# darglein/Snake-SLAM

Measured on AMD Instinct MI355X. Metric: frames/s ORB extract+match @752x480, higher is better.
Workload: dtype u8

## Files before the change

### include/snake_hip.h

```cpp
#ifndef SNAKE_HIP_H
#define SNAKE_HIP_H

#include <stddef.h>
#include <stdint.h>

#ifdef __cplusplus
extern "C" {
#endif

#define SNK_API __attribute__((visibility("default")))

typedef enum snk_status
{
    SNK_OK                = 0,
    SNK_ERR_INVALID_ARG   = 1,
    SNK_ERR_NO_DEVICE     = 2,
    SNK_ERR_HIP           = 3,
    SNK_ERR_CAPACITY      = 4,
    SNK_ERR_NOT_CONFIGURED = 5,
    SNK_ERR_TIMEOUT       = 6
} snk_status;

#define SNK_DIST_INF 256

// ... 84 lines not shown
                                     int out_cap);

SNK_API int snk_orb_set_profiling(snk_orb* o, int enable);

SNK_API int snk_orb_set_chains(snk_orb* o, int chains);
SNK_API int snk_orb_set_stagger(snk_orb* o, int parts);
SNK_API int snk_orb_stage_times(snk_orb* o, float* ms, int* n_calls);

enum
{
    SNK_ORB_DEBUG_PYRAMID         = 1,
    SNK_ORB_DEBUG_CELL_COUNTS     = 2,
    SNK_ORB_DEBUG_CELL_CANDIDATES = 3,
    SNK_ORB_DEBUG_SELECTED        = 4,
    SNK_ORB_DEBUG_SELECTED_COUNT  = 5,
    SNK_ORB_DEBUG_LEVEL_INFO      = 6
};
SNK_API int snk_orb_debug_fetch(snk_orb* o, int what, int image, int level, void* out, size_t cap_bytes,
                                size_t* n_bytes);


typedef struct snk_rectification
{
    double K_src[4];
    double D_src[8];
    double R[9];
    double K_dst[4];
    double bf;
} snk_rectification;

SNK_API int snk_rectify(snk_matcher* m, const snk_rectification* rect, const snk_keypoint* kps, int n, snk_kp64* out,
// ... 557 lines not shown
```

### snake_slam_amd/csrc/orb.hip

```cpp
#include "common.hpp"

#include <array>
#include <vector>

namespace snk
{
namespace
{
using u8  = unsigned char;
using u16 = unsigned short;
using u32 = unsigned int;
using u64 = unsigned long long;

constexpr int MAX_LEVELS     = 16;
constexpr int EDGE_THRESHOLD = 19;
constexpr int MIN_BORDER     = 16;
constexpr int CELL_W         = 30;
constexpr int CELL_SLOTS     = 64;
constexpr int KEY_DIGITS     = 16;
constexpr int DEFAULT_LEVEL_CAP = 8192;
#ifndef SNK_DIST_MIN_WAVES
#define SNK_DIST_MIN_WAVES 1
#endif
#ifndef SNK_FAST_MIN_WAVES
// ... 1056 lines not shown
                    }
                    if (out_lane && !no_blur_store)
                    {
                        const u32 lo = __builtin_amdgcn_perm(a[1], a[0], 0x0c0c0602u);
                        const u32 hi = __builtin_amdgcn_perm(a[3], a[2], 0x06020c0cu);
                        *reinterpret_cast<u32*>(blur + (blur_tiled ? blur_tiled_y(yo, bpitch) : (u32)(yo * bpitch)) + xl_store) = lo | hi;
                    }
                }
#pragma unroll
                for (int c = 0; c < 4; ++c) pr[kk][c] = __builtin_amdgcn_alignbit(hc[c], pr[(kk + 6) % 7][c], 16);
            }
        }
    }
}

__device__ __forceinline__ u64 point_key(int x, int y, int W, int H, int nroots)
{
    const u32 ux = (u32)x, uw = (u32)W, un = (u32)nroots;
    const int root = (int)((ux * un) / uw);
    int x0 = (int)(((u32)root * uw + un - 1u) / un), x1 = (int)(((u32)(root + 1) * uw + un - 1u) / un);
    int y0 = 0, y1 = H;
    u64 key = (u64)root;
    const int ext = max(max(W, H), 2);
    const int nd  = min(KEY_DIGITS, 32 - __clz(ext - 1));
    for (int d = 0; d < nd; ++d)
    {
        const int mx = x0 + (x1 - x0 + 1) / 2, my = y0 + (y1 - y0 + 1) / 2;
        const int cx = x >= mx, cy = y >= my;
        x0 = cx ? mx : x0;
        x1 = cx ? x1 : mx;
        y0 = cy ? my : y0;
        y1 = cy ? y1 : my;
        key = (key << 2) | (u64)(cx + 2 * cy);
    }
    return key << (2 * (KEY_DIGITS - nd));
}

__device__ void bitonic_sort(u64* a, int n_pow2, int tid, int nthreads)
{
    const int nw = nthreads >> 6, wave = tid >> 6, lane = tid & 63;
    const int seg = n_pow2 / nw;
    if (seg < 128)
    {
        for (int k = 2; k <= n_pow2; k <<= 1)
            for (int j = k >> 1; j > 0; j >>= 1)
            {
                for (int t = tid; t < (n_pow2 >> 1); t += nthreads)
                {
                    const int i   = ((t & ~(j - 1)) << 1) | (t & (j - 1));
                    const int ixj = i | j;
// ... 39 lines not shown
                const bool up = (i & k) == 0;
                const u64 x = a[i], y = a[ixj];
                if ((x > y) == up)
                {
                    a[i]   = y;
                    a[ixj] = x;
                }
            }
            __builtin_amdgcn_wave_barrier();
        }
    }
    __syncthreads();
}

constexpr int DIST_THREADS = 512;
__device__ int block_scan_incl(int v, int tid, int* wave_tot )
{
    const int lane = tid & 63, wave = tid >> 6;
    int x = v;
    x = wave_scan_incl_dpp(x);
    if (lane == 63) wave_tot[wave] = x;
    __syncthreads();
    int base = 0;
    for (int w = 0; w < wave; ++w) base += wave_tot[w];
    __syncthreads();
    return x + base;
}

__device__ void bucket_rank_sort(u64* keys, int n, int cap, int nroots, unsigned char* tmp, int tid, int* wave_tot)
{
    u16* idx  = reinterpret_cast<u16*>(tmp);
    int* hist = reinterpret_cast<int*>(tmp + 2 * cap);
    const int nb_max = min(1023, cap / 2 - 1);
    int T = 4;
    while (T > 0 && (nroots << (2 * T)) > nb_max) --T;
    const int nb    = nroots << (2 * T);
    const int shift = 13 + 32 - 2 * T;
    for (int i = tid; i <= nb; i += DIST_THREADS) hist[i] = 0;
    __syncthreads();
    for (int i = tid; i < n; i += DIST_THREADS) atomicAdd(&hist[(int)(keys[i] >> shift)], 1);
    __syncthreads();
    {
        const int b0 = 2 * tid, c0 = b0 < nb ? hist[b0] : 0, c1 = b0 + 1 < nb ? hist[b0 + 1] : 0;
        const int incl = block_scan_incl(c0 + c1, tid, wave_tot);
        if (b0 < nb) hist[b0] = incl - c0 - c1;
        if (b0 + 1 < nb) hist[b0 + 1] = incl - c1;
    }
    __syncthreads();
    for (int i = tid; i < n; i += DIST_THREADS) idx[atomicAdd(&hist[(int)(keys[i] >> shift)], 1)] = (u16)i;
    __syncthreads();
    u64 mine[4];
    int dest[4];
#pragma unroll
    for (int u = 0; u < 4; ++u)
    {
        const int i = tid + u * DIST_THREADS;
        mine[u] = 0;
        dest[u] = -1;
        if (i < n)
// ... 15 lines not shown
    }
    __syncthreads();
#pragma unroll
    for (int u = 0; u < 4; ++u)
        if (dest[u] >= 0) keys[dest[u]] = mine[u];
    __syncthreads();
}

__device__ bool distribute_body(const Layout& L, int b, int l, int lds_cap, u32* cand ,
                                const u16* __restrict__ cell_cnt, u32* __restrict__ sel ,
                                u8* __restrict__ sel_score, int* __restrict__ sel_cnt,
                                int* __restrict__ cand_total ,
                                unsigned long long* __restrict__ dbg_t = nullptr ,
                                u32* cand_h = nullptr ,
                                u32* __restrict__ sel_resp = nullptr ,
                                u32* __restrict__ h_global = nullptr )
{
    extern __shared__ __attribute__((aligned(16))) unsigned char smem[];
    const int cap     = lds_cap;
    const int sem_cap = L.level_cap;
    u64* keys     = reinterpret_cast<u64*>(smem);
    u64* nodes    = keys + cap;
    u16* px       = reinterpret_cast<u16*>(nodes + cap / 2);
    u16* py       = px + cap;
    u8* sc        = reinterpret_cast<u8*>(py + cap);
    signed char* lcp = reinterpret_cast<signed char*>(sc + cap);
    u8* fd        = reinterpret_cast<u8*>(lcp + cap + 16);
    u32* hv       = cand_h ? (h_global ? h_global : reinterpret_cast<u32*>(smem + ((cap * 8 + cap / 2 * 8 + cap * 2 * 2 + cap + (cap + 16) + cap + 15) & ~15)))
                           : nullptr;
    __shared__ int wave_tot[8];
    __shared__ int hist_lcp[20], hist_m[20];
    __shared__ int s_n, s_k, s_D, s_careful, s_size, s_nnodes, s_finish, s_jstar, s_out;

    const int tid = threadIdx.x;
    unsigned long long t_prev = dbg_t ? __builtin_readcyclecounter() : 0ull;
    auto mark = [&](int phase)
    {
        if (dbg_t && tid == 0)
        {
            const unsigned long long t = __builtin_readcyclecounter();
            atomicAdd(&dbg_t[l * 16 + phase], t - t_prev);
            t_prev = t;
        }
    };
    const LevelInfo& lv = L.lv[l];
    const int ncell = lv.ncols * lv.nrows;
    const int N     = lv.nfeat;
    const u16* cc   = cell_cnt + (long long)b * L.total_cells + lv.cell_off;
    u32* cd         = cand + ((long long)b * L.total_cells + lv.cell_off) * CELL_SLOTS;
    u32* chd        = cand_h ? cand_h + ((long long)b * L.total_cells + lv.cell_off) * CELL_SLOTS : nullptr;
    int* out_cnt    = sel_cnt + b * MAX_LEVELS + l;

    if (tid == 0) s_k = CELL_SLOTS;
    __syncthreads();
    for (;;)
    {
        const int k = s_k;
        int part    = 0;
        for (int c = tid; c < ncell; c += DIST_THREADS) part += min((int)cc[c], k);
        const int incl = block_scan_incl(part, tid, wave_tot);
        if (tid == DIST_THREADS - 1) s_n = incl;
        __syncthreads();
        if (s_n <= sem_cap || k == 0) break;
        if (tid == 0) s_k = k - 1;
        __syncthreads();
    }
    const int kcell = s_k;
    const int n     = s_n;
    mark(0);
    if (n > cap) return false;
    if (kcell < CELL_SLOTS)
    {
        u32* cdw = cd;
        u32* chw = chd;
        const int lane = tid & 63;
        for (int c = tid >> 6; c < ncell; c += DIST_THREADS / 64)
        {
            const int cnt = (int)cc[c];
            if (cnt <= kcell || cnt > CELL_SLOTS) continue;
            const u32 k = lane < cnt ? cdw[(long long)c * CELL_SLOTS + lane] : 0u;
            const u32 h = chw && lane < cnt ? chw[(long long)c * CELL_SLOTS + lane] : 0u;
            int r       = 0;
            for (int j = 0; j < cnt; ++j) r += (u32)__builtin_amdgcn_readlane((int)k, __builtin_amdgcn_readfirstlane(j)) > k ? 1 : 0;
// ... 8 lines not shown
    }
    if (tid == 0 && cand_total) cand_total[b * MAX_LEVELS + l] = n;
    if (n == 0 || N <= 0)
    {
        if (tid == 0) *out_cnt = 0;
        return true;
    }
    int n_pow2 = 1;
    while (n_pow2 < n) n_pow2 <<= 1;

    {
        int base = 0;
        for (int c0 = 0; c0 < ncell; c0 += DIST_THREADS)
        {
            const int c   = c0 + tid;
            const int cnt = c < ncell ? min((int)cc[c], kcell) : 0;
            const int incl = block_scan_incl(cnt, tid, wave_tot);
            const int off  = base + incl - cnt;
            if (cnt > 0)
            {
                const int ci = c / lv.ncols, cj = c - ci * lv.ncols;
                const int x0 = EDGE_THRESHOLD + cj * lv.wcell, y0 = EDGE_THRESHOLD + ci * lv.hcell;
                const uint4* cq = reinterpret_cast<const uint4*>(cd + (long long)c * CELL_SLOTS);
                for (int i = 0; i < cnt; i += 32)
                {
                    uint4 q[8];
#pragma unroll
                    for (int v = 0; v < 8; ++v) q[v] = i + 4 * v < cnt ? cq[(i >> 2) + v] : uint4{0u, 0u, 0u, 0u};
#pragma unroll
                    for (int v = 0; v < 8; ++v)
                    {
                        const u32 kk[4] = {q[v].x, q[v].y, q[v].z, q[v].w};
#pragma unroll
                        for (int u = 0; u < 4; ++u)
                            if (i + 4 * v + u < cnt)
                            {
                                const u32 k = kk[u];
                                const int o = off + i + 4 * v + u;
                                px[o] = (u16)(x0 + 63 - (int)(k & 63u));
                                py[o] = (u16)(y0 + 63 - (int)((k >> 6) & 63u));
                                sc[o] = (u8)(k >> 12);
                                if (hv) hv[o] = chd[(long long)c * CELL_SLOTS + i + 4 * v + u];
                            }
                    }
                }
            }
            if (tid == DIST_THREADS - 1) s_out = incl;
            __syncthreads();
            base += s_out;
            __syncthreads();
        }
    }
    mark(1);
    const int W = lv.w - 2 * MIN_BORDER, H = lv.h - 2 * MIN_BORDER;
    for (int i = tid; i < n_pow2; i += DIST_THREADS)
        keys[i] = i < n ? ((point_key(px[i] - MIN_BORDER, py[i] - MIN_BORDER, W, H, lv.nroots) << 13) | (u64)i) : ~0ull;
    __syncthreads();

    mark(2);
    if (n <= 4 * DIST_THREADS && cap >= 512)
        bucket_rank_sort(keys, n, cap, lv.nroots, reinterpret_cast<unsigned char*>(nodes), tid, wave_tot);
    else
        bitonic_sort(keys, n_pow2, tid, DIST_THREADS);
    mark(3);

    if (tid < 20)
    {
        hist_lcp[tid] = 0;
        hist_m[tid]   = 0;
    }
    for (int i = tid; i <= n; i += DIST_THREADS)
    {
        int v = -1;
        if (i > 0 && i < n)
        {
            const u64 diff = (keys[i] >> 13) ^ (keys[i - 1] >> 13);
// ... 31 lines not shown
            const int multi = size - cum_m;
            if (size >= N || size == size_prev)
            {
                D = d; careful = 0; size_D = size; done = true;
            }
            else if (size + 3 * multi > N)
            {
                D = d; careful = 1; size_D = size; done = true;
            }
            size_prev = size;
            if (!done && d == KEY_DIGITS) { D = KEY_DIGITS; careful = 0; size_D = size; }
        }
        s_D       = D;
        s_careful = careful;
        s_size    = size_D;
        s_finish  = 0;
    }
    __syncthreads();
    const int D = s_D;
    for (int i = tid; i < n; i += DIST_THREADS) fd[i] = (u8)D;
    __syncthreads();

    mark(5);
    if (s_careful && n <= 4 * DIST_THREADS)
    {
        int* hist = reinterpret_cast<int*>(nodes);
        const int HN = n - 1;
        for (int dd = D; dd < KEY_DIGITS; ++dd)
        {
            for (int k = tid; k < HN; k += DIST_THREADS) hist[k] = 0;
            if (tid == 0) s_jstar = HN;
            if (dbg_t && tid == 0) atomicAdd(&dbg_t[l * 16 + 14], 1ull);
            __syncthreads();
            int cntv[4], delv[4];
            bool any = false;
#pragma unroll
            for (int u = 0; u < 4; ++u)
            {
                const int i = 4 * tid + u;
                cntv[u] = delv[u] = 0;
                if (i < n && fd[i] == dd && (int)lcp[i] < dd)
                {
                    int e = i + 1, delta = 0;
                    for (;;)
                    {
                        const int l0 = lcp[e], l1 = lcp[e + 1], l2 = lcp[e + 2], l3 = lcp[e + 3];
// ... 13 lines not shown
                }
            }
            mark(8);
            if (!__syncthreads_or(any ? 1 : 0)) break;
            mark(9);
            int before_mine = 0;
            {
                int loc[4], sum = 0;
#pragma unroll
                for (int u = 0; u < 4; ++u)
                {
                    const int k = 4 * tid + u;
                    loc[u]      = k < HN ? hist[HN - 1 - k] : 0;
                    sum += loc[u];
                }
                const int incl = block_scan_incl(sum, tid, wave_tot);
                int run        = s_size + incl - sum;
                int found      = -1;
#pragma unroll
                for (int u = 0; u < 4; ++u)
                {
                    if (found < 0 && loc[u] > 0 && run + loc[u] >= N) { found = 4 * tid + u; before_mine = run; }
                    run += loc[u];
                }
                if (found >= 0) atomicMin(&s_jstar, found);
                if (tid == DIST_THREADS - 1) s_out = run - s_size;
            }
            __syncthreads();
            mark(10);
            const int kstar = s_jstar;
            if (kstar < HN && 4 * tid <= kstar && kstar < 4 * tid + 4) s_nnodes = before_mine;
            __syncthreads();
            const int cstar  = kstar < HN ? HN - 1 - kstar + 2 : 0;
            const int before = kstar < HN ? s_nnodes : 0;
            int my_add = 0;
            bool split[4];
#pragma unroll
            for (int u = 0; u < 4; ++u) split[u] = cntv[u] > 0 && (cstar == 0 || cntv[u] > cstar);
            if (cstar != 0)
            {
                int d[4], sum = 0;
#pragma unroll
                for (int u = 0; u < 4; ++u)
                {
                    d[u] = cntv[u] == cstar ? delv[u] : 0;
                    sum += d[u];
                }
                int run = before + block_scan_incl(sum, tid, wave_tot) - sum;
#pragma unroll
                for (int u = 0; u < 4; ++u)
                {
                    if (cntv[u] == cstar && run < N) split[u] = true;
                    run += d[u];
                }
            }
#pragma unroll
            for (int u = 0; u < 4; ++u)
                if (split[u]) my_add += delv[u];
            mark(11);
            const int add = block_scan_incl(my_add, tid, wave_tot);
            if (tid == DIST_THREADS - 1)
            {
                s_finish = (s_size + add >= N || add == 0) ? 1 : 0;
                s_size += add;
            }
#pragma unroll
            for (int u = 0; u < 4; ++u)
                if (split[u])
                    for (int e = 4 * tid + u, e1 = e + cntv[u]; e < e1; ++e) fd[e] = (u8)(dd + 1);
            __syncthreads();
            mark(12);
            if (s_finish) break;
        }
    }
    else if (s_careful)
    {
        for (int dd = D; dd < KEY_DIGITS; ++dd)
        {
            if (tid == 0) s_nnodes = 0;
            __syncthreads();
            for (int i = tid; i < n; i += DIST_THREADS)
            {
                if (fd[i] != dd || (int)lcp[i] >= dd) continue;
                int e = i + 1, delta = 0;
                while (e < n && (int)lcp[e] >= dd)
                {
                    delta += (int)lcp[e] == dd ? 1 : 0;
// ... 4 lines not shown
                {
                    const u64 nk = ((u64)(0xFFFF - cnt) << 32) | ((u64)i << 16) | (u64)delta;
                    nodes[atomicAdd(&s_nnodes, 1)] = nk;
                }
            }
            __syncthreads();
            const int m = s_nnodes;
            if (m == 0) break;
            int m_pow2 = 1;
            while (m_pow2 < m) m_pow2 <<= 1;
            for (int i = m + tid; i < m_pow2; i += DIST_THREADS) nodes[i] = ~0ull;
            __syncthreads();
            bitonic_sort(nodes, m_pow2, tid, DIST_THREADS);
            if (tid == 0) s_jstar = m;
            __syncthreads();
            int base = s_size;
            for (int j0 = 0; j0 < m; j0 += DIST_THREADS)
            {
                const int j     = j0 + tid;
                const int delta = j < m ? (int)(nodes[j] & 0xFFFFu) : 0;
                const int incl  = block_scan_incl(delta, tid, wave_tot);
                if (j < m && base + incl >= N) atomicMin(&s_jstar, j);
                if (tid == DIST_THREADS - 1) s_out = incl;
                __syncthreads();
                base += s_out;
                __syncthreads();
            }
            const int jstar = s_jstar;
            const int last  = jstar < m ? jstar : m - 1;
            {
                int part = 0;
                for (int j = tid; j <= last; j += DIST_THREADS) part += (int)(nodes[j] & 0xFFFFu);
                const int add = block_scan_incl(part, tid, wave_tot);
                if (tid == DIST_THREADS - 1)
                {
                    s_finish = (s_size + add >= N || add == 0) ? 1 : 0;
                    s_size += add;
                }
            }
            for (int j = tid; j <= last; j += DIST_THREADS)
            {
                const int i = (int)((nodes[j] >> 16) & 0xFFFFu);
                int e       = i;
                do
                {
                    fd[e] = (u8)(dd + 1);
                    ++e;
                } while (e < n && (int)lcp[e] >= dd);
            }
            __syncthreads();
            if (s_finish) break;
        }
    }
    __syncthreads();

    mark(6);
    {
        u32* out    = sel + (long long)b * L.total_slots + lv.slot_off;
        u8* out_sc  = sel_score + (long long)b * L.total_slots + lv.slot_off;
        for (int i = tid; i < n; i += DIST_THREADS)
        {
            const int c = (int)(keys[i] & 0x1FFFu);
            keys[i]     = ((u64)(hv ? hv[c] : (u32)sc[c]) << 32) | ((u64)(0xFFFFu - py[c]) << 16) | (u64)(0xFFFFu - px[c]);
        }
        __syncthreads();
        unsigned long long* best = reinterpret_cast<unsigned long long*>(nodes);
        const int best_cap = min(n, lv.slot_cap);
        for (int k = tid; k < best_cap; k += DIST_THREADS) best[k] = 0ull;
        __syncthreads();
        int base = 0;
        for (int i0 = 0; i0 < n; i0 += DIST_THREADS)
        {
            const int i     = i0 + tid;
            const bool head = i < n && (int)lcp[i] < (int)fd[i];
            const int incl  = block_scan_incl(head ? 1 : 0, tid, wave_tot);
            const int pos   = base + incl - 1;
            if (i < n && pos < best_cap) atomicMax(&best[pos], (unsigned long long)keys[i]);
            if (tid == DIST_THREADS - 1) s_out = incl;
            __syncthreads();
            base += s_out;
            __syncthreads();
        }
        const int count = base < lv.slot_cap ? base : lv.slot_cap;
        for (int k = tid; k < count; k += DIST_THREADS)
        {
            const unsigned long long w = best[k];
            out[k]    = (0xFFFFu - (u32)(w & 0xFFFFu)) | ((0xFFFFu - (u32)((w >> 16) & 0xFFFFu)) << 16);
            out_sc[k] = (u8)(w >> 32);
            if (sel_resp) sel_resp[(long long)b * L.total_slots + lv.slot_off + k] = (u32)(w >> 32);
        }
        if (tid == 0) *out_cnt = count;
    }
    mark(7);
    if (dbg_t && tid == 0) atomicAdd(&dbg_t[l * 16 + 15], (unsigned long long)n);
    return true;
}

__global__ __launch_bounds__(DIST_THREADS, SNK_DIST_MIN_WAVES) void distribute_kernel(Layout L, int lds_cap, u32* cand,
                                                                  const u16* __restrict__ cell_cnt, u32* __restrict__ sel,
                                                                  u8* __restrict__ sel_score, int* __restrict__ sel_cnt,
                                                                  int* __restrict__ cand_total, int* __restrict__ queue,
                                                                  unsigned long long* __restrict__ dbg_t, u32* cand_h,
                                                                  u32* __restrict__ sel_resp)
{
    const int l = blockIdx.x, b = blockIdx.y;
    if (!distribute_body(L, b, l, lds_cap, cand, cell_cnt, sel, sel_score, sel_cnt, cand_total, dbg_t, cand_h, sel_resp) && threadIdx.x == 0)
        queue[1 + atomicAdd(&queue[0], 1)] = b * MAX_LEVELS + l;
}

__global__ __launch_bounds__(DIST_THREADS) void distribute_large_kernel(Layout L, u32* cand,
                                                                        const u16* __restrict__ cell_cnt,
                                                                        u32* __restrict__ sel, u8* __restrict__ sel_score,
                                                                        int* __restrict__ sel_cnt, int* __restrict__ cand_total,
                                                                        const int* __restrict__ queue, u32* cand_h,
                                                                        u32* __restrict__ sel_resp, u32* __restrict__ h_scratch)
{
    const int count = queue[0];
    for (int i = blockIdx.x; i < count; i += gridDim.x)
    {
        const int item = queue[1 + i];
        distribute_body(L, item / MAX_LEVELS, item % MAX_LEVELS, L.level_cap, cand, cell_cnt, sel, sel_score, sel_cnt, cand_total, nullptr,
                        cand_h, sel_resp, cand_h ? h_scratch + (size_t)blockIdx.x * L.level_cap : nullptr);
        __syncthreads();
    }
}

__device__ __forceinline__ float fast_atan2_deg(float y, float x)
{
    const float p1 = 0x1.ca44dep+5f, p3 = -0x1.2aaddcp+4f, p5 = 0x1.1d3f7ep+3f, p7 = -0x1.4515b2p+1f;
    const float ax = fabsf(x), ay = fabsf(y);
    float a, c, c2;
    if (ax >= ay)
    {
        c  = ay / (ax + 0x1p-52f);
        c2 = c * c;
        a  = (((p7 * c2 + p5) * c2 + p3) * c2 + p1) * c;
    }
// ... 439 lines not shown
}
}

using namespace snk;

struct snk_orb : HandleBase
{
    snk_orb_params params{};
    int width = 0, height = 0, max_batch = 0;
    bool configured = false;
    Layout lay{};
    DevBuf pyr[MAX_LEVELS];
    DevBuf blur[MAX_LEVELS];
    DevBuf tables;
    DevBuf cell_tab;
    DevBuf img0;
    DevBuf cand, cell_cnt, sel, sel_score, sel_cnt, cand_total, dist_queue;
    DevBuf cand_h, sel_resp, dist_h;
    DevBuf out_kps;
    HostBuf h_out, h_img;
    int pitch0_host = 0;
    size_t dist_lds = 0, dist_lds_small = 0;
    int dist_small_cap = 0;
    bool profiling = false;
    std::vector<std::array<hipEvent_t, 7>> ev_sets;
    size_t ev_used = 0;
    static constexpr int MAX_PARTS = 4;
    hipStream_t stream2 = nullptr;
    hipStream_t extra[MAX_PARTS - 1] = {nullptr, nullptr, nullptr};
    hipEvent_t ev_fork = nullptr, ev_join_n[MAX_PARTS - 1] = {nullptr, nullptr, nullptr};
// ... 37 lines not shown
        const int width = lv.w - 2 * MIN_BORDER, height = lv.h - 2 * MIN_BORDER;
        lv.ncols = width > 0 ? width / CELL_W : 0;
        lv.nrows = height > 0 ? height / CELL_W : 0;
        if (lv.ncols < 1 || lv.nrows < 1 || lv.w < 2 * EDGE_THRESHOLD + 1 || lv.h < 2 * EDGE_THRESHOLD + 1)
        {
            lv.ncols = lv.nrows = 0;
            lv.wcell = lv.hcell = 1;
        }
        else
        {
            lv.wcell = (width + lv.ncols - 1) / lv.ncols;
            lv.hcell = (height + lv.nrows - 1) / lv.nrows;
        }
        lv.cell_off = cell_off;
        cell_off += lv.ncols * lv.nrows;
        int nroots = height > 0 ? (2 * width + height) / (2 * height) : 1;
        nroots     = nroots < 1 ? 1 : (nroots > 255 ? 255 : nroots);
        lv.nroots  = nroots;
        lv.slot_off = slot_off;
        lv.slot_cap = lv.nfeat + 3 > 4 * nroots ? lv.nfeat + 3 : 4 * nroots;
        slot_off += lv.slot_cap;
        lv.pitch      = (lv.w + 63) & ~63;
        lv.img_stride = (long long)lv.pitch * lv.h;
        lv.blur_stride = (long long)lv.pitch * ((lv.h + 3) & ~3);
        if (lv.w > 0 && lv.h > 0)
        {
            static const bool balanced = getenv("SNK_ORB_BALANCED_STRIPS") != nullptr;
            if (balanced || lv.w <= 4 * SM_LANES_OUT)
            {
                lv.n_strips     = ceil_div(lv.w, 4 * SM_LANES_OUT);
                lv.strip_stride = ((ceil_div(lv.w, lv.n_strips) + 3) / 4) * 4;
            }
            else
// ... 123 lines not shown
    *out = o;
    return SNK_OK;
}

int snk_orb_destroy(snk_orb* o)
{
    if (!o) return SNK_OK;
    (void)hipSetDevice(o->device);
    for (auto& b : o->pyr) b.release();
    for (auto& b : o->blur) b.release();
    o->tables.release();
    o->img0.release();
    o->cand.release();
    o->cell_cnt.release();
    o->cell_tab.release();
    o->sel.release();
    o->sel_score.release();
    o->sel_cnt.release();
    o->cand_total.release();
    o->dist_queue.release();
    o->cand_h.release();
    o->sel_resp.release();
    o->dist_h.release();
    o->out_kps.release();
    o->h_out.release();
    o->h_img.release();
    for (auto& e : o->ev_sets)
        for (auto& x : e) (void)hipEventDestroy(x);
    if (o->ev_fork) (void)hipEventDestroy(o->ev_fork);
    for (auto& e : o->ev_front)
// ... 88 lines not shown
                const int ci = c / lv.ncols, cj = c - ci * lv.ncols;
                const int x0 = EDGE_THRESHOLD + cj * lv.wcell, y0 = EDGE_THRESHOLD + ci * lv.hcell;
                const int x1 = std::min(x0 + lv.wcell, lv.w - EDGE_THRESHOLD), y1 = std::min(y0 + lv.hcell, lv.h - EDGE_THRESHOLD);
                int4 e;
                e.x = x0;
                e.y = y0;
                e.z = (int)(((unsigned)(x1 - x0) & 0xFFFFu) | ((unsigned)(y1 - y0) << 16));
                e.w = l;
                ct[(size_t)lv.cell_off + c] = e;
            }
        }
        if ((rc = o->cell_tab.reserve(ct.size() * sizeof(int4))) != SNK_OK) return rc;
        if ((rc = copy_sync(o->cell_tab.p, ct.data(), ct.size() * sizeof(int4), hipMemcpyHostToDevice, o->stream)) != SNK_OK) return rc;
        L.cell_tab = o->cell_tab.as<int4>();
    }
    const size_t cells = (size_t)(L.total_cells > 0 ? L.total_cells : 1) * max_batch;
    const size_t slots = (size_t)(L.total_slots > 0 ? L.total_slots : 1) * max_batch;
    if ((rc = o->cand.reserve(cells * CELL_SLOTS * sizeof(u32))) != SNK_OK) return rc;
    if ((rc = o->cell_cnt.reserve(cells * sizeof(u16))) != SNK_OK) return rc;
    if ((rc = o->sel.reserve(slots * sizeof(u32))) != SNK_OK) return rc;
    if ((rc = o->sel_score.reserve(slots)) != SNK_OK) return rc;
    if ((rc = o->sel_cnt.reserve((size_t)max_batch * MAX_LEVELS * sizeof(int))) != SNK_OK) return rc;
    if ((rc = o->cand_total.reserve((size_t)max_batch * MAX_LEVELS * sizeof(int))) != SNK_OK) return rc;
    auto dist_lds_bytes = [](size_t cap) { return cap * 8 + cap / 2 * 8 + cap * 2 * 2 + cap + (cap + 16) + cap; };
    o->dist_small_cap = L.level_cap < 2048 ? L.level_cap : 2048;
    o->dist_lds       = dist_lds_bytes((size_t)L.level_cap);
    o->dist_lds_small = dist_lds_bytes((size_t)o->dist_small_cap);
    if ((rc = o->dist_queue.reserve(snk_orb::MAX_PARTS * ((size_t)max_batch * MAX_LEVELS + 1) * sizeof(int))) != SNK_OK) return rc;
    SNK_REQUIRE(4 * L.f_lds_wave <= LDS_MAX_BYTES, "FAST cells too large for the LDS (image too small for its cell grid?)");
    if ((rc = set_max_lds_once(reinterpret_cast<const void*>(distribute_kernel), (int)std::max(dist_lds_bytes(2048) + 4 * 2048 + 16, dist_lds_bytes(8192)))) != SNK_OK) return rc;
// ... 142 lines not shown
        static const size_t lds_wg_env = getenv("SNK_ORB_FAST_LDS_WG") ? (size_t)atoll(getenv("SNK_ORB_FAST_LDS_WG")) : 0;
        const size_t fast_lds = std::max((size_t)4 * L.f_lds_wave, std::min(lds_wg_env, (size_t)LDS_MAX_BYTES));
        hipLaunchKernelGGL(fk, xcd_grid(gx, batch), dim3(256), fast_lds, st, L, images_dev, pitch,
                           image_stride, aligned0, o->params.ini_th_fast, o->params.min_th_fast, d_cand, d_cellcnt, gx, batch, fast_stop,
                           cpw, stages == 3 ? d_queue : (int*)nullptr);
        SNK_LAUNCH_CHECK();
    }
    if (ev) SNK_HIP_CHECK(hipEventRecord((*ev)[3], st));
    }
    if (!(stages & 2)) return SNK_OK;
    if (ev) SNK_HIP_CHECK(hipEventRecord((*ev)[6], st));
    {
    const int aligned0 = (reinterpret_cast<uintptr_t>(images_dev) % 4 == 0 && pitch % 4 == 0 && image_stride % 4 == 0) ? 1 : 0;
    if (stages != 3 || L.total_cells <= 0) SNK_HIP_CHECK(hipMemsetAsync(d_queue, 0, sizeof(int), st));
    static const bool dist_timing = getenv("SNK_ORB_DIST_TIMING") != nullptr;
    unsigned long long* d_dbg = nullptr;
    if (dist_timing)
    {
        SNK_HIP_CHECK(hipMalloc(&d_dbg, MAX_LEVELS * 16 * sizeof(unsigned long long)));
        SNK_HIP_CHECK(hipMemsetAsync(d_dbg, 0, MAX_LEVELS * 16 * sizeof(unsigned long long), st));
    }
    if (harris && L.total_cells > 0)
    {
        static const bool per_cell = getenv("SNK_ORB_HARRIS_PER_CELL") != nullptr;
        if (per_cell)
        {
            const int gxh = ceil_div(L.total_cells, 4);
            hipLaunchKernelGGL(harris_kernel, xcd_grid(gxh, batch), dim3(256), 0, st, L, images_dev, pitch, image_stride, aligned0, d_cand, d_cellcnt,
                               d_candh, gxh, batch);
        }
        else
        {
            const int gxh = ceil_div(ceil_div(L.total_cells, HARRIS_NC), 4);
            hipLaunchKernelGGL(harris_dense_kernel, xcd_grid(gxh, batch), dim3(256), 0, st, L, images_dev, pitch, image_stride, aligned0, d_cand,
                               d_cellcnt, d_candh, gxh, batch);
        }
        SNK_LAUNCH_CHECK();
    }
    const bool one_dist_launch = !harris && o->dist_small_cap < L.level_cap && (long long)L.n_levels * batch <= 128;
    hipLaunchKernelGGL(distribute_kernel, dim3(L.n_levels, batch), dim3(DIST_THREADS),
                       one_dist_launch ? o->dist_lds : o->dist_lds_small + (harris ? 4 * (size_t)o->dist_small_cap + 16 : 0), st, L,
                       one_dist_launch ? L.level_cap : o->dist_small_cap, d_cand, d_cellcnt, d_sel, d_selscore,
                       d_selcnt, d_candtot, d_queue, d_dbg, d_candh, d_selresp);
    SNK_LAUNCH_CHECK();
    if (dist_timing)
    {
        unsigned long long h[MAX_LEVELS * 16];
        SNK_HIP_CHECK(hipStreamSynchronize(st));
        SNK_HIP_CHECK(hipMemcpy(h, d_dbg, sizeof(h), hipMemcpyDeviceToHost));
        SNK_HIP_CHECK(hipFree(d_dbg));
        for (int l = 0; l < L.n_levels; ++l)
        {
            fprintf(stderr, "[dist timing] level %d (avg candidates %.0f, %.2f careful rounds), cycles per workgroup:", l,
                    (double)h[l * 16 + 15] / batch, (double)h[l * 16 + 14] / batch);
            for (int ph = 0; ph < 13; ++ph) fprintf(stderr, " %.0f", (double)h[l * 16 + ph] / batch);
            fprintf(stderr, "\n");
        }
    }
    if (o->dist_small_cap < L.level_cap && !one_dist_launch)
    {
        hipLaunchKernelGGL(distribute_large_kernel, dim3(large_workers), dim3(DIST_THREADS), o->dist_lds, st, L,
                           d_cand, d_cellcnt, d_sel, d_selscore,
                           d_selcnt, d_candtot, d_queue, d_candh, d_selresp, d_disth);
        SNK_LAUNCH_CHECK();
    }
    if (ev) SNK_HIP_CHECK(hipEventRecord((*ev)[4], st));
    int max_slot = 1;
    for (int l = 0; l < L.n_levels; ++l) max_slot = L.lv[l].slot_cap > max_slot ? L.lv[l].slot_cap : max_slot;
    {
        const int nb = batch >= 16 ? 8 * ceil_div(batch, 8) : batch;
        static const bool blur_in = getenv("SNK_ORB_BLUR_IN_DESCRIBE") != nullptr;
        static const bool dma = getenv("SNK_ORB_DESC_NO_DMA") == nullptr;
        const int dfake       = getenv("SNK_ORB_DESC_FAKE") ? atoi(getenv("SNK_ORB_DESC_FAKE")) : 0;
        const int gx          = ceil_div(max_slot, 4 * DESC_KPW);
        auto dk = describe_kernel<false, false, false>;
        if (blur_in) dk = describe_kernel<true, false, false>;
        else if (dma && orb_blur_mode() == 2) dk = describe_kernel<false, true, true>;
        else if (dma) dk = describe_kernel<false, true, false>;
// ... 206 lines not shown
            src   = o->cell_cnt.as<u16>() + (long long)image * L.total_cells + lv.cell_off;
            bytes = (size_t)lv.ncols * lv.nrows * sizeof(u16);
            break;
        case SNK_ORB_DEBUG_CELL_CANDIDATES:
            src   = o->cand.as<u32>() + ((long long)image * L.total_cells + lv.cell_off) * CELL_SLOTS;
            bytes = (size_t)lv.ncols * lv.nrows * CELL_SLOTS * sizeof(u32);
            break;
        case SNK_ORB_DEBUG_SELECTED:
            src   = o->sel.as<u32>() + (long long)image * L.total_slots + lv.slot_off;
            bytes = (size_t)lv.slot_cap * sizeof(u32);
            break;
        case SNK_ORB_DEBUG_SELECTED_COUNT:
            src   = o->sel_cnt.as<int>() + image * MAX_LEVELS + level;
            bytes = sizeof(int);
            break;
        case SNK_ORB_DEBUG_LEVEL_INFO:
        {
            int info[8] = {lv.w, lv.h, lv.pitch, lv.ncols, lv.nrows, lv.wcell, lv.hcell, lv.nfeat};
            SNK_REQUIRE(cap_bytes >= sizeof(info), "buffer too small");
            memcpy(out, info, sizeof(info));
            *n_bytes = sizeof(info);
            return SNK_OK;
        }
        default: SNK_REQUIRE(false, "unknown debug selector");
    }
    SNK_REQUIRE(out != nullptr && cap_bytes >= bytes, "buffer too small");
    if (int rc = copy_sync(out, src, bytes, hipMemcpyDeviceToHost, o->stream)) return rc;
    *n_bytes = bytes;
    return SNK_OK;
}
// ... 2 lines not shown
```

### snake_slam_amd/orb.py

```python
from __future__ import annotations

import ctypes as C

import numpy as np

from . import _lib

KEYPOINT_DTYPE = np.dtype([("x", "<f4"), ("y", "<f4"), ("size", "<f4"), ("angle", "<f4"), ("response", "<f4"),
                           ("octave", "<i4")])

DEBUG_PYRAMID, DEBUG_CELL_COUNTS, DEBUG_CELL_CANDIDATES, DEBUG_SELECTED, DEBUG_SELECTED_COUNT, DEBUG_LEVEL_INFO = range(1, 7)


class OrbParams(C.Structure):
    _fields_ = [("nfeatures", C.c_int32), ("scale_factor", C.c_float), ("n_levels", C.c_int32),
                ("ini_th_fast", C.c_int32), ("min_th_fast", C.c_int32), ("level_cap", C.c_int32)]


class ORBExtractor:
    def __init__(self, nfeatures: int = 1000, scale_factor: float = 1.2, n_levels: int = 4, ini_th_fast: int = 20,
                 min_th_fast: int = 7, level_cap: int = 0, device: int = 0, stream: int | None = None):
        self._lib = _lib.load()
        self.params = OrbParams(nfeatures, scale_factor, n_levels, ini_th_fast, min_th_fast, level_cap)
        h = C.c_void_p()
        _lib.check(self._lib.snk_orb_create(C.byref(self.params), device, C.c_void_p(stream or 0), C.byref(h)),
                   "snk_orb_create")
# ... 71 lines not shown
```

Measured before the change: 193,000.

## Use precomputed key tables and barrier-light block scans in distribute kernel

Replaces the per-point quadtree key loop with lookups into per-level x/y digit tables built on the host at configure time, then combines them by bit interleaving. Block scans now double-buffer the wave totals and return the block total to every thread, which removes many shared-variable broadcasts and extra __syncthreads in the count, compaction and node-splitting loops. The jstar search packs the index and prefix into one atomicMin to drop another barrier round. This adds a small device table and relies on the table-derived keys matching the loop-derived keys exactly.

```diff
diff --git a/include/snake_hip.h b/include/snake_hip.h
--- a/include/snake_hip.h
+++ b/include/snake_hip.h
@@ -122,7 +122,8 @@
     SNK_ORB_DEBUG_CELL_CANDIDATES = 3,
     SNK_ORB_DEBUG_SELECTED        = 4,
     SNK_ORB_DEBUG_SELECTED_COUNT  = 5,
-    SNK_ORB_DEBUG_LEVEL_INFO      = 6
+    SNK_ORB_DEBUG_LEVEL_INFO      = 6,
+    SNK_ORB_DEBUG_DIST_QUEUE      = 7
 };
 SNK_API int snk_orb_debug_fetch(snk_orb* o, int what, int image, int level, void* out, size_t cap_bytes,
                                 size_t* n_bytes);
diff --git a/snake_slam_amd/csrc/orb.hip b/snake_slam_amd/csrc/orb.hip
--- a/snake_slam_amd/csrc/orb.hip
+++ b/snake_slam_amd/csrc/orb.hip
@@ -1,4 +1,5 @@
 #include "common.hpp"
+#include "orb_keys.hpp"
 
 #include <array>
 #include <vector>
@@ -1094,26 +1095,10 @@
     }
 }
 
-__device__ __forceinline__ u64 point_key(int x, int y, int W, int H, int nroots)
-{
-    const u32 ux = (u32)x, uw = (u32)W, un = (u32)nroots;
-    const int root = (int)((ux * un) / uw);
-    int x0 = (int)(((u32)root * uw + un - 1u) / un), x1 = (int)(((u32)(root + 1) * uw + un - 1u) / un);
-    int y0 = 0, y1 = H;
-    u64 key = (u64)root;
-    const int ext = max(max(W, H), 2);
-    const int nd  = min(KEY_DIGITS, 32 - __clz(ext - 1));
-    for (int d = 0; d < nd; ++d)
-    {
-        const int mx = x0 + (x1 - x0 + 1) / 2, my = y0 + (y1 - y0 + 1) / 2;
-        const int cx = x >= mx, cy = y >= my;
-        x0 = cx ? mx : x0;
-        x1 = cx ? x1 : mx;
-        y0 = cy ? my : y0;
-        y1 = cy ? y1 : my;
-        key = (key << 2) | (u64)(cx + 2 * cy);
-    }
-    return key << (2 * (KEY_DIGITS - nd));
+__device__ __forceinline__ u64 point_key(int x, int y, int W, int H, int nroots, const u32* __restrict__ keyx, const u32* __restrict__ keyy)
+{
+    if (keyx) return orb_key_from_tables(keyx[x], keyy[y]);
+    return orb_point_key(x, y, W, H, nroots);
 }
 
 __device__ void bitonic_sort(u64* a, int n_pow2, int tid, int nthreads)
@@ -1183,20 +1168,32 @@
 }
 
 constexpr int DIST_THREADS = 512;
-__device__ int block_scan_incl(int v, int tid, int* wave_tot )
+struct ScanBuf
+{
+    int4 tot[2][2];
+};
+__device__ __forceinline__ int block_scan_incl(int v, int tid, ScanBuf& sb, int& par, int& total)
 {
     const int lane = tid & 63, wave = tid >> 6;
     int x = v;
     x = wave_scan_incl_dpp(x);
-    if (lane == 63) wave_tot[wave] = x;
+    if (lane == 63) reinterpret_cast<int*>(sb.tot[par])[wave] = x;
     __syncthreads();
-    int base = 0;
-    for (int w = 0; w < wave; ++w) base += wave_tot[w];
-    __syncthreads();
+    const int4 a = sb.tot[par][0], b = sb.tot[par][1];
+    par ^= 1;
+    const int t[8] = {a.x, a.y, a.z, a.w, b.x, b.y, b.z, b.w};
+    int base = 0, sum = 0;
+#pragma unroll
+    for (int w = 0; w < 8; ++w)
+    {
+        base += w < wave ? t[w] : 0;
+        sum += t[w];
+    }
+    total = __builtin_amdgcn_readfirstlane(sum);
     return x + base;
 }
 
-__device__ void bucket_rank_sort(u64* keys, int n, int cap, int nroots, unsigned char* tmp, int tid, int* wave_tot)
+__device__ void bucket_rank_sort(u64* keys, int n, int cap, int nroots, unsigned char* tmp, int tid, ScanBuf& sb, int& par)
 {
     u16* idx  = reinterpret_cast<u16*>(tmp);
     int* hist = reinterpret_cast<int*>(tmp + 2 * cap);
@@ -1211,7 +1208,8 @@
     __syncthreads();
     {
         const int b0 = 2 * tid, c0 = b0 < nb ? hist[b0] : 0, c1 = b0 + 1 < nb ? hist[b0 + 1] : 0;
-        const int incl = block_scan_incl(c0 + c1, tid, wave_tot);
+        int total;
+        const int incl = block_scan_incl(c0 + c1, tid, sb, par, total);
         if (b0 < nb) hist[b0] = incl - c0 - c1;
         if (b0 + 1 < nb) hist[b0 + 1] = incl - c1;
     }
@@ -1257,7 +1255,8 @@
                                 unsigned long long* __restrict__ dbg_t = nullptr ,
                                 u32* cand_h = nullptr ,
                                 u32* __restrict__ sel_resp = nullptr ,
-                                u32* __restrict__ h_global = nullptr )
+                                u32* __restrict__ h_global = nullptr ,
+                                const u32* __restrict__ key_tab = nullptr )
 {
     extern __shared__ __attribute__((aligned(16))) unsigned char smem[];
     const int cap     = lds_cap;
@@ -1271,9 +1270,10 @@
     u8* fd        = reinterpret_cast<u8*>(lcp + cap + 16);
     u32* hv       = cand_h ? (h_global ? h_global : reinterpret_cast<u32*>(smem + ((cap * 8 + cap / 2 * 8 + cap * 2 * 2 + cap + (cap + 16) + cap + 15) & ~15)))
                            : nullptr;
-    __shared__ int wave_tot[8];
+    __shared__ ScanBuf sb;
     __shared__ int hist_lcp[20], hist_m[20];
-    __shared__ int s_n, s_k, s_D, s_careful, s_size, s_nnodes, s_finish, s_jstar, s_out;
+    __shared__ int s_D, s_careful, s_size, s_nnodes, s_jstar;
+    int par = 0, total;
 
     const int tid = threadIdx.x;
     unsigned long long t_prev = dbg_t ? __builtin_readcyclecounter() : 0ull;
@@ -1294,22 +1294,17 @@
     u32* chd        = cand_h ? cand_h + ((long long)b * L.total_cells + lv.cell_off) * CELL_SLOTS : nullptr;
     int* out_cnt    = sel_cnt + b * MAX_LEVELS + l;
 
-    if (tid == 0) s_k = CELL_SLOTS;
-    __syncthreads();
+    const int cnt0 = tid < ncell ? (int)cc[tid] : 0;
+    int kcell = CELL_SLOTS, n;
     for (;;)
     {
-        const int k = s_k;
-        int part    = 0;
-        for (int c = tid; c < ncell; c += DIST_THREADS) part += min((int)cc[c], k);
-        const int incl = block_scan_incl(part, tid, wave_tot);
-        if (tid == DIST_THREADS - 1) s_n = incl;
-        __syncthreads();
-        if (s_n <= sem_cap || k == 0) break;
-        if (tid == 0) s_k = k - 1;
-        __syncthreads();
-    }
-    const int kcell = s_k;
-    const int n     = s_n;
+        int part = min(cnt0, kcell);
+        for (int c = tid + DIST_THREADS; c < ncell; c += DIST_THREADS) part += min((int)cc[c], kcell);
+        block_scan_incl(part, tid, sb, par, total);
+        n = total;
+        if (n <= sem_cap || kcell == 0) break;
+        --kcell;
+    }
     mark(0);
     if (n > cap) return false;
     if (kcell < CELL_SLOTS)
@@ -1348,8 +1343,8 @@
         for (int c0 = 0; c0 < ncell; c0 += DIST_THREADS)
         {
             const int c   = c0 + tid;
-            const int cnt = c < ncell ? min((int)cc[c], kcell) : 0;
-            const int incl = block_scan_incl(cnt, tid, wave_tot);
+            const int cnt = c0 == 0 ? min(cnt0, kcell) : (c < ncell ? min((int)cc[c], kcell) : 0);
+            const int incl = block_scan_incl(cnt, tid, sb, par, total);
             const int off  = base + incl - cnt;
             if (cnt > 0)
             {
@@ -1379,21 +1374,38 @@
                     }
                 }
             }
-            if (tid == DIST_THREADS - 1) s_out = incl;
-            __syncthreads();
-            base += s_out;
-            __syncthreads();
-        }
+            base += total;
+        }
+        __syncthreads();
     }
     mark(1);
     const int W = lv.w - 2 * MIN_BORDER, H = lv.h - 2 * MIN_BORDER;
-    for (int i = tid; i < n_pow2; i += DIST_THREADS)
-        keys[i] = i < n ? ((point_key(px[i] - MIN_BORDER, py[i] - MIN_BORDER, W, H, lv.nroots) << 13) | (u64)i) : ~0ull;
+    {
+        const u32* keyx = key_tab ? key_tab + key_tab[l] : nullptr;
+        const u32* keyy = key_tab ? keyx + max(W, 0) : nullptr;
+        constexpr int KEY_ILP = 4;
+        for (int i0 = tid; i0 < n_pow2; i0 += KEY_ILP * DIST_THREADS)
+        {
+            u64 k[KEY_ILP];
+#pragma unroll
+            for (int u = 0; u < KEY_ILP; ++u)
+            {
+                const int i = i0 + u * DIST_THREADS;
+                k[u] = i < n ? ((point_key(px[i] - MIN_BORDER, py[i] - MIN_BORDER, W, H, lv.nroots, keyx, keyy) << 13) | (u64)i) : ~0ull;
+            }
+#pragma unroll
+            for (int u = 0; u < KEY_ILP; ++u)
+            {
+                const int i = i0 + u * DIST_THREADS;
+                if (i < n_pow2) keys[i] = k[u];
+            }
+        }
+    }
     __syncthreads();
 
     mark(2);
     if (n <= 4 * DIST_THREADS && cap >= 512)
-        bucket_rank_sort(keys, n, cap, lv.nroots, reinterpret_cast<unsigned char*>(nodes), tid, wave_tot);
+        bucket_rank_sort(keys, n, cap, lv.nroots, reinterpret_cast<unsigned char*>(nodes), tid, sb, par);
     else
         bitonic_sort(keys, n_pow2, tid, DIST_THREADS);
     mark(3);
@@ -1455,10 +1467,10 @@
         s_D       = D;
         s_careful = careful;
         s_size    = size_D;
-        s_finish  = 0;
     }
     __syncthreads();
     const int D = s_D;
+    int size    = s_size;
     for (int i = tid; i < n; i += DIST_THREADS) fd[i] = (u8)D;
     __syncthreads();
 
@@ -1470,7 +1482,7 @@
         for (int dd = D; dd < KEY_DIGITS; ++dd)
         {
             for (int k = tid; k < HN; k += DIST_THREADS) hist[k] = 0;
-            if (tid == 0) s_jstar = HN;
+            if (tid == 0) s_jstar = HN << 16;
             if (dbg_t && tid == 0) atomicAdd(&dbg_t[l * 16 + 14], 1ull);
             __syncthreads();
             int cntv[4], delv[4];
@@ -1514,8 +1526,8 @@
                     loc[u]      = k < HN ? hist[HN - 1 - k] : 0;
                     sum += loc[u];
                 }
-                const int incl = block_scan_incl(sum, tid, wave_tot);
-                int run        = s_size + incl - sum;
+                const int incl = block_scan_incl(sum, tid, sb, par, total);
+                int run        = size + incl - sum;
                 int found      = -1;
 #pragma unroll
                 for (int u = 0; u < 4; ++u)
@@ -1523,16 +1535,14 @@
                     if (found < 0 && loc[u] > 0 && run + loc[u] >= N) { found = 4 * tid + u; before_mine = run; }
                     run += loc[u];
                 }
-                if (found >= 0) atomicMin(&s_jstar, found);
-                if (tid == DIST_THREADS - 1) s_out = run - s_size;
+                if (found >= 0) atomicMin(&s_jstar, (found << 16) | before_mine);
             }
             __syncthreads();
             mark(10);
-            const int kstar = s_jstar;
-            if (kstar < HN && 4 * tid <= kstar && kstar < 4 * tid + 4) s_nnodes = before_mine;
-            __syncthreads();
+            const int jst    = s_jstar;
+            const int kstar  = jst >> 16;
             const int cstar  = kstar < HN ? HN - 1 - kstar + 2 : 0;
-            const int before = kstar < HN ? s_nnodes : 0;
+            const int before = kstar < HN ? (jst & 0xFFFF) : 0;
             int my_add = 0;
             bool split[4];
 #pragma unroll
@@ -1546,7 +1556,7 @@
                     d[u] = cntv[u] == cstar ? delv[u] : 0;
                     sum += d[u];
                 }
-                int run = before + block_scan_incl(sum, tid, wave_tot) - sum;
+                int run = before + block_scan_incl(sum, tid, sb, par, total) - sum;
 #pragma unroll
                 for (int u = 0; u < 4; ++u)
                 {
@@ -1558,19 +1568,17 @@
             for (int u = 0; u < 4; ++u)
                 if (split[u]) my_add += delv[u];
             mark(11);
-            const int add = block_scan_incl(my_add, tid, wave_tot);
-            if (tid == DIST_THREADS - 1)
-            {
-                s_finish = (s_size + add >= N || add == 0) ? 1 : 0;
-                s_size += add;
-            }
+            block_scan_incl(my_add, tid, sb, par, total);
+            const int add     = total;
+            const bool finish = size + add >= N || add == 0;
+            size += add;
 #pragma unroll
             for (int u = 0; u < 4; ++u)
                 if (split[u])
                     for (int e = 4 * tid + u, e1 = e + cntv[u]; e < e1; ++e) fd[e] = (u8)(dd + 1);
             __syncthreads();
             mark(12);
-            if (s_finish) break;
+            if (finish) break;
         }
     }
     else if (s_careful)
@@ -1605,29 +1613,25 @@
             bitonic_sort(nodes, m_pow2, tid, DIST_THREADS);
             if (tid == 0) s_jstar = m;
             __syncthreads();
-            int base = s_size;
+            int base = size;
             for (int j0 = 0; j0 < m; j0 += DIST_THREADS)
             {
                 const int j     = j0 + tid;
                 const int delta = j < m ? (int)(nodes[j] & 0xFFFFu) : 0;
-                const int incl  = block_scan_incl(delta, tid, wave_tot);
+                const int incl  = block_scan_incl(delta, tid, sb, par, total);
                 if (j < m && base + incl >= N) atomicMin(&s_jstar, j);
-                if (tid == DIST_THREADS - 1) s_out = incl;
-                __syncthreads();
-                base += s_out;
-                __syncthreads();
-            }
+                base += total;
+            }
+            __syncthreads();
             const int jstar = s_jstar;
             const int last  = jstar < m ? jstar : m - 1;
+            bool finish;
             {
                 int part = 0;
                 for (int j = tid; j <= last; j += DIST_THREADS) part += (int)(nodes[j] & 0xFFFFu);
-                const int add = block_scan_incl(part, tid, wave_tot);
-                if (tid == DIST_THREADS - 1)
-                {
-                    s_finish = (s_size + add >= N || add == 0) ? 1 : 0;
-                    s_size += add;
-                }
+                block_scan_incl(part, tid, sb, par, total);
+                finish = size + total >= N || total == 0;
+                size += total;
             }
             for (int j = tid; j <= last; j += DIST_THREADS)
             {
@@ -1640,7 +1644,7 @@
                 } while (e < n && (int)lcp[e] >= dd);
             }
             __syncthreads();
-            if (s_finish) break;
+            if (finish) break;
         }
     }
     __syncthreads();
@@ -1664,14 +1668,12 @@
         {
             const int i     = i0 + tid;
             const bool head = i < n && (int)lcp[i] < (int)fd[i];
-            const int incl  = block_scan_incl(head ? 1 : 0, tid, wave_tot);
+            const int incl  = block_scan_incl(head ? 1 : 0, tid, sb, par, total);
             const int pos   = base + incl - 1;
             if (i < n && pos < best_cap) atomicMax(&best[pos], (unsigned long long)keys[i]);
-            if (tid == DIST_THREADS - 1) s_out = incl;
-            __syncthreads();
-            base += s_out;
-            __syncthreads();
-        }
+            base += total;
+        }
+        __syncthreads();
         const int count = base < lv.slot_cap ? base : lv.slot_cap;
         for (int k = tid; k < count; k += DIST_THREADS)
         {
@@ -1692,10 +1694,11 @@
                                                                   u8* __restrict__ sel_score, int* __restrict__ sel_cnt,
                                                                   int* __restrict__ cand_total, int* __restrict__ queue,
                                                                   unsigned long long* __restrict__ dbg_t, u32* cand_h,
-                                                                  u32* __restrict__ sel_resp)
+                                                                  u32* __restrict__ sel_resp, const u32* __restrict__ key_tab)
 {
     const int l = blockIdx.x, b = blockIdx.y;
-    if (!distribute_body(L, b, l, lds_cap, cand, cell_cnt, sel, sel_score, sel_cnt, cand_total, dbg_t, cand_h, sel_resp) && threadIdx.x == 0)
+    if (!distribute_body(L, b, l, lds_cap, cand, cell_cnt, sel, sel_score, sel_cnt, cand_total, dbg_t, cand_h, sel_resp, nullptr, key_tab) &&
+        threadIdx.x == 0)
         queue[1 + atomicAdd(&queue[0], 1)] = b * MAX_LEVELS + l;
 }
 
@@ -1704,14 +1707,15 @@
                                                                         u32* __restrict__ sel, u8* __restrict__ sel_score,
                                                                         int* __restrict__ sel_cnt, int* __restrict__ cand_total,
                                                                         const int* __restrict__ queue, u32* cand_h,
-                                                                        u32* __restrict__ sel_resp, u32* __restrict__ h_scratch)
+                                                                        u32* __restrict__ sel_resp, u32* __restrict__ h_scratch,
+                                                                        const u32* __restrict__ key_tab)
 {
     const int count = queue[0];
     for (int i = blockIdx.x; i < count; i += gridDim.x)
     {
         const int item = queue[1 + i];
         distribute_body(L, item / MAX_LEVELS, item % MAX_LEVELS, L.level_cap, cand, cell_cnt, sel, sel_score, sel_cnt, cand_total, nullptr,
-                        cand_h, sel_resp, cand_h ? h_scratch + (size_t)blockIdx.x * L.level_cap : nullptr);
+                        cand_h, sel_resp, cand_h ? h_scratch + (size_t)blockIdx.x * L.level_cap : nullptr, key_tab);
         __syncthreads();
     }
 }
@@ -2181,6 +2185,7 @@
     DevBuf blur[MAX_LEVELS];
     DevBuf tables;
     DevBuf cell_tab;
+    DevBuf key_tab;
     DevBuf img0;
     DevBuf cand, cell_cnt, sel, sel_score, sel_cnt, cand_total, dist_queue;
     DevBuf cand_h, sel_resp, dist_h;
@@ -2248,9 +2253,8 @@
         }
         lv.cell_off = cell_off;
         cell_off += lv.ncols * lv.nrows;
-        int nroots = height > 0 ? (2 * width + height) / (2 * height) : 1;
-        nroots     = nroots < 1 ? 1 : (nroots > 255 ? 255 : nroots);
-        lv.nroots  = nroots;
+        const int nroots = orb_key_nroots(width, height);
+        lv.nroots        = nroots;
         lv.slot_off = slot_off;
         lv.slot_cap = lv.nfeat + 3 > 4 * nroots ? lv.nfeat + 3 : 4 * nroots;
         slot_off += lv.slot_cap;
@@ -2404,6 +2408,7 @@
     o->cand.release();
     o->cell_cnt.release();
     o->cell_tab.release();
+    o->key_tab.release();
     o->sel.release();
     o->sel_score.release();
     o->sel_cnt.release();
@@ -2522,6 +2527,20 @@
         if ((rc = copy_sync(o->cell_tab.p, ct.data(), ct.size() * sizeof(int4), hipMemcpyHostToDevice, o->stream)) != SNK_OK) return rc;
         L.cell_tab = o->cell_tab.as<int4>();
     }
+    {
+        std::vector<u32> kt(MAX_LEVELS, 0u);
+        for (int l = 0; l < L.n_levels; ++l)
+        {
+            const LevelInfo& lv = L.lv[l];
+            const int W = std::max(lv.w - 2 * MIN_BORDER, 0), H = std::max(lv.h - 2 * MIN_BORDER, 0);
+            kt[l] = (u32)kt.size();
+            if (W == 0 || H == 0) continue;
+            for (int x = 0; x < W; ++x) kt.push_back(orb_keyx_entry(x, W, H, lv.nroots));
+            for (int y = 0; y < H; ++y) kt.push_back(orb_keyy_entry(y, W, H));
+        }
+        if ((rc = o->key_tab.reserve(kt.size() * sizeof(u32))) != SNK_OK) return rc;
+        if ((rc = copy_sync(o->key_tab.p, kt.data(), kt.size() * sizeof(u32), hipMemcpyHostToDevice, o->stream)) != SNK_OK) return rc;
+    }
     const size_t cells = (size_t)(L.total_cells > 0 ? L.total_cells : 1) * max_batch;
     const size_t slots = (size_t)(L.total_slots > 0 ? L.total_slots : 1) * max_batch;
     if ((rc = o->cand.reserve(cells * CELL_SLOTS * sizeof(u32))) != SNK_OK) return rc;
@@ -2694,6 +2713,8 @@
     const int aligned0 = (reinterpret_cast<uintptr_t>(images_dev) % 4 == 0 && pitch % 4 == 0 && image_stride % 4 == 0) ? 1 : 0;
     if (stages != 3 || L.total_cells <= 0) SNK_HIP_CHECK(hipMemsetAsync(d_queue, 0, sizeof(int), st));
     static const bool dist_timing = getenv("SNK_ORB_DIST_TIMING") != nullptr;
+    static const bool key_loop    = getenv("SNK_ORB_DIST_KEY_LOOP") != nullptr;
+    const u32* d_keytab           = key_loop ? nullptr : o->key_tab.as<u32>();
     unsigned long long* d_dbg = nullptr;
     if (dist_timing)
     {
@@ -2721,7 +2742,7 @@
     hipLaunchKernelGGL(distribute_kernel, dim3(L.n_levels, batch), dim3(DIST_THREADS),
                        one_dist_launch ? o->dist_lds : o->dist_lds_small + (harris ? 4 * (size_t)o->dist_small_cap + 16 : 0), st, L,
                        one_dist_launch ? L.level_cap : o->dist_small_cap, d_cand, d_cellcnt, d_sel, d_selscore,
-                       d_selcnt, d_candtot, d_queue, d_dbg, d_candh, d_selresp);
+                       d_selcnt, d_candtot, d_queue, d_dbg, d_candh, d_selresp, d_keytab);
     SNK_LAUNCH_CHECK();
     if (dist_timing)
     {
@@ -2741,7 +2762,7 @@
     {
         hipLaunchKernelGGL(distribute_large_kernel, dim3(large_workers), dim3(DIST_THREADS), o->dist_lds, st, L,
                            d_cand, d_cellcnt, d_sel, d_selscore,
-                           d_selcnt, d_candtot, d_queue, d_candh, d_selresp, d_disth);
+                           d_selcnt, d_candtot, d_queue, d_candh, d_selresp, d_disth, d_keytab);
         SNK_LAUNCH_CHECK();
     }
     if (ev) SNK_HIP_CHECK(hipEventRecord((*ev)[4], st));
@@ -2978,6 +2999,10 @@
             src   = o->sel_cnt.as<int>() + image * MAX_LEVELS + level;
             bytes = sizeof(int);
             break;
+        case SNK_ORB_DEBUG_DIST_QUEUE:
+            src   = o->dist_queue.as<int>();
+            bytes = ((size_t)o->max_batch * MAX_LEVELS + 1) * sizeof(int);
+            break;
         case SNK_ORB_DEBUG_LEVEL_INFO:
         {
             int info[8] = {lv.w, lv.h, lv.pitch, lv.ncols, lv.nrows, lv.wcell, lv.hcell, lv.nfeat};
diff --git a/snake_slam_amd/csrc/orb_keys.hpp b/snake_slam_amd/csrc/orb_keys.hpp
--- /dev/null
+++ b/snake_slam_amd/csrc/orb_keys.hpp
@@ -0,0 +1,94 @@
+#pragma once
+#include <cstdint>
+
+#if defined(__HIPCC__) || defined(__CUDACC__)
+#define SNK_KEYS_HD __host__ __device__ inline
+#else
+#define SNK_KEYS_HD inline
+#endif
+
+namespace snk
+{
+constexpr int ORB_KEY_DIGITS = 16;
+
+SNK_KEYS_HD int orb_key_ndigits(int W, int H)
+{
+    int ext = W > H ? W : H;
+    if (ext < 2) ext = 2;
+    const int nd = 32 - __builtin_clz((unsigned)(ext - 1));
+    return nd < ORB_KEY_DIGITS ? nd : ORB_KEY_DIGITS;
+}
+
+SNK_KEYS_HD int orb_key_root(int x, int W, int nroots) { return (int)(((uint32_t)x * (uint32_t)nroots) / (uint32_t)W); }
+SNK_KEYS_HD int orb_key_root_begin(int root, int W, int nroots)
+{
+    return (int)(((uint32_t)root * (uint32_t)W + (uint32_t)nroots - 1u) / (uint32_t)nroots);
+}
+
+SNK_KEYS_HD uint32_t orb_key_axis_digits(int v, int lo, int hi, int nd)
+{
+    uint32_t bits = 0;
+    for (int d = 0; d < nd; ++d)
+    {
+        const int m = lo + (hi - lo + 1) / 2;
+        const int c = v >= m;
+        lo          = c ? m : lo;
+        hi          = c ? hi : m;
+        bits        = (bits << 1) | (uint32_t)c;
+    }
+    return bits;
+}
+
+SNK_KEYS_HD uint32_t orb_keyx_entry(int x, int W, int H, int nroots)
+{
+    const int nd = orb_key_ndigits(W, H), root = orb_key_root(x, W, nroots);
+    const uint32_t bits = orb_key_axis_digits(x, orb_key_root_begin(root, W, nroots), orb_key_root_begin(root + 1, W, nroots), nd);
+    return ((uint32_t)root << 16) | (bits << (ORB_KEY_DIGITS - nd));
+}
+SNK_KEYS_HD uint32_t orb_keyy_entry(int y, int W, int H)
+{
+    const int nd = orb_key_ndigits(W, H);
+    return orb_key_axis_digits(y, 0, H, nd) << (ORB_KEY_DIGITS - nd);
+}
+
+SNK_KEYS_HD uint32_t orb_key_spread16(uint32_t v)
+{
+    v &= 0xFFFFu;
+    v = (v | (v << 8)) & 0x00FF00FFu;
+    v = (v | (v << 4)) & 0x0F0F0F0Fu;
+    v = (v | (v << 2)) & 0x33333333u;
+    v = (v | (v << 1)) & 0x55555555u;
+    return v;
+}
+
+SNK_KEYS_HD uint64_t orb_key_from_tables(uint32_t kx, uint32_t ky)
+{
+    return ((uint64_t)(kx >> 16) << 32) | (uint64_t)(orb_key_spread16(kx) | (orb_key_spread16(ky) << 1));
+}
+
+SNK_KEYS_HD uint64_t orb_point_key(int x, int y, int W, int H, int nroots)
+{
+    const int root = orb_key_root(x, W, nroots);
+    int x0 = orb_key_root_begin(root, W, nroots), x1 = orb_key_root_begin(root + 1, W, nroots);
+    int y0 = 0, y1 = H;
+    uint64_t key = (uint64_t)root;
+    const int nd = orb_key_ndigits(W, H);
+    for (int d = 0; d < nd; ++d)
+    {
+        const int mx = x0 + (x1 - x0 + 1) / 2, my = y0 + (y1 - y0 + 1) / 2;
+        const int cx = x >= mx, cy = y >= my;
+        x0  = cx ? mx : x0;
+        x1  = cx ? x1 : mx;
+        y0  = cy ? my : y0;
+        y1  = cy ? y1 : my;
+        key = (key << 2) | (uint64_t)(cx + 2 * cy);
+    }
+    return key << (2 * (ORB_KEY_DIGITS - nd));
+}
+
+SNK_KEYS_HD int orb_key_nroots(int W, int H)
+{
+    int n = H > 0 ? (2 * W + H) / (2 * H) : 1;
+    return n < 1 ? 1 : (n > 255 ? 255 : n);
+}
+}
diff --git a/snake_slam_amd/orb.py b/snake_slam_amd/orb.py
--- a/snake_slam_amd/orb.py
+++ b/snake_slam_amd/orb.py
@@ -10,6 +10,7 @@
                            ("octave", "<i4")])
 
 DEBUG_PYRAMID, DEBUG_CELL_COUNTS, DEBUG_CELL_CANDIDATES, DEBUG_SELECTED, DEBUG_SELECTED_COUNT, DEBUG_LEVEL_INFO = range(1, 7)
+DEBUG_DIST_QUEUE = 7
 
 
 class OrbParams(C.Structure):
```

Result: faster. 195,700, median of 6 (+1.4%).
